# namascar/correlation

Hardware: AMD Instinct MI355X
Metric: correlation-point-iterations/sec (higher is better)
Workload: dtype f32

## Files before the change

### correlation_amd/build.py

```python
import os
import subprocess
import sys

HERE = os.path.dirname(os.path.abspath(__file__))
CSRC = os.path.join(HERE, "csrc")
LIB = os.path.join(HERE, "liblk_engine.so")
SOURCES = ["lk_engine.cpp", "lk_tracker.cpp", "lk_group.cpp", "lk_image_io.cpp", "lk_kernels.hip", "lk_guess_search.cpp",
           "lk_guess_search.hip", "lk_backward.hip", "lk_reseed.cpp", "lk_reseed.hip",
           "lk_strain.cpp", "lk_strain.hip", "lk_uncertainty.cpp", "lk_uncertainty.hip",
           "lk_outlier.cpp", "lk_outlier.hip", "lk_track.cpp", "lk_track.hip",
           "lk_residual.cpp", "lk_residual.hip", "lk_pattern.cpp", "lk_pattern.hip",
           "lk_field.cpp", "lk_field.hip", "lk_znssd.cpp", "lk_znssd.hip"]
HEADERS = ["lk_device.hpp", "lk_roi.hpp", "lk_solver_common.hpp", "lk_compose.hpp", "lk_launch.hpp", "lk_neighbours.hpp", "lk_rect_walk.hpp", "lk_sector_eval.hpp", "lk_cell_grid.hpp", "lk_pass.hpp", "lk_strain.hpp", "lk_uncertainty.hpp", "lk_outlier.hpp", "lk_track.hpp", "lk_residual.hpp", "lk_pattern.hpp", "lk_field.hpp", "lk_znssd.hpp", os.path.join("..", "..", "include", "lk_engine.h"),
           os.path.join("..", "..", "include", "lk_tracker.h"), os.path.join("..", "..", "include", "lk_group.h")]


def hipcc_path():
    for cand in (os.environ.get("HIPCC"), "/opt/rocm/bin/hipcc", "hipcc"):
        if cand and (os.path.isabs(cand) and os.path.exists(cand) or not os.path.isabs(cand)):
            return cand
    raise RuntimeError("hipcc not found")


def needs_build():
    if not os.path.exists(LIB):
        return True
    t = os.path.getmtime(LIB)
    deps = [os.path.join(CSRC, f) for f in SOURCES + HEADERS] + [os.path.abspath(__file__)]
    return any(os.path.getmtime(d) > t for d in deps if os.path.exists(d))


def build(force=False, verbose=False):
    if not force and not needs_build():
        return LIB
    from concurrent.futures import ThreadPoolExecutor
    objdir = os.path.join(os.path.dirname(HERE), "build", "obj")
    os.makedirs(objdir, exist_ok=True)
    flags = [
        "-O3", "--offload-arch=gfx950", "-fPIC", "-std=c++17",
        "-ffp-contract=off", "-fhip-fp32-correctly-rounded-divide-sqrt",
        "-fno-slp-vectorize",
        "-Wall", "-Wextra",
    ] + os.environ.get("LK_EXTRA_HIPCC_FLAGS", "").split()
    if verbose:
        flags.insert(0, "-Rpass-analysis=kernel-resource-usage")
    tag = os.path.join(objdir, "flags.txt")
    same_flags = os.path.exists(tag) and open(tag).read() == " ".join(flags)
    hdr_time = max(os.path.getmtime(os.path.join(CSRC, h)) for h in HEADERS + ["lk_internal.hpp"] if os.path.exists(os.path.join(CSRC, h)))

    def compile_one(src):
        obj = os.path.join(objdir, src + ".o")
        src_path = os.path.join(CSRC, src)
        if (not force and same_flags and os.path.exists(obj)
                and os.path.getmtime(obj) > max(os.path.getmtime(src_path), hdr_time)):
            return obj, None
        r = subprocess.run([hipcc_path()] + flags + ["-c", src, "-o", obj], cwd=CSRC, capture_output=True, text=True)
        return obj, r

    with ThreadPoolExecutor(max_workers=len(SOURCES)) as pool:
        results = list(pool.map(compile_one, SOURCES))
    for obj, r in results:
        if r is not None and r.returncode != 0:
            sys.stderr.write(r.stdout + r.stderr)
            raise RuntimeError("hipcc failed building " + os.path.basename(obj))
        if r is not None and verbose:
            sys.stderr.write(r.stderr)
    with open(tag, "w") as f:
        f.write(" ".join(flags))
    link = [hipcc_path(), "--offload-arch=gfx950", "-fPIC", "-shared", "-o", LIB] + [o for o, _ in results] + [
        "-lrocprofiler-sdk-roctx",
        "-lrccl",
        "-lz",
    ]
    r = subprocess.run(link, cwd=CSRC, capture_output=True, text=True)
    if r.returncode != 0:
        sys.stderr.write(r.stdout + r.stderr)
        raise RuntimeError("hipcc failed linking liblk_engine.so")
    return LIB


if __name__ == "__main__":
    print(build(force="--force" in sys.argv, verbose="-v" in sys.argv))
```

### correlation_amd/csrc/lk_kernels.hip

```cpp
#include "lk_device.hpp"
#include "lk_launch.hpp"

#include <float.h>
#include <stdlib.h>

#include <atomic>

#include "lk_rect_walk.hpp"
#include "lk_solver_common.hpp"

namespace {

struct LevelCtx {
  gptr<uint8_t> und, def;
  gptr<f32x2> xy;
  int rx, ry, rw;
  int n;
  int urows, ucols, drows, dcols;
  float cx, cy, scaling;
};

__device__ __forceinline__ float row16_sum(float v) {
  v = dpp_add<0xB1>(v);
  v = dpp_add<0x4E>(v);
// ... 1999 lines not shown
#pragma unroll
    for (int k = 0; k < 6; ++k)
      pr[k] = ps[k] = q[30 + k];
    const bool fr = damped_step<6, false>(S, lambda, scaling, pr, false, xr);
    const bool fs = damped_step_scattered(q[mine], q[mine + 1], lambda, scaling, ps, xs);
    bool same = __builtin_amdgcn_readfirstlane((int)fs) == (int)fs;
#pragma unroll
    for (int k = 0; k < 6; ++k)
      same = same && __builtin_amdgcn_readfirstlane((int)__float_as_uint(xs[k])) == (int)__float_as_uint(xs[k]) &&
             __builtin_amdgcn_readfirstlane((int)__float_as_uint(ps[k])) == (int)__float_as_uint(ps[k]);
    const bool all_same = __ballot(same) == ~0ull;
    if (l == 0) {
      float *o = out + (size_t)i * 32;
#pragma unroll
      for (int k = 0; k < 6; ++k) {
        o[k] = xr[k];
        o[6 + k] = pr[k];
        o[16 + k] = xs[k];
        o[22 + k] = ps[k];
      }
      o[12] = fr ? 1.f : 0.f;
      o[28] = fs ? 1.f : 0.f;
      o[13] = o[14] = o[15] = o[30] = o[31] = 0.f;
      o[29] = all_same ? 1.f : 0.f;
    }
  }
}

template <int N> __device__ __forceinline__ void row16_all_reduce(float (&v)[N]) {
#pragma unroll
  for (int i = 0; i < N; ++i)
    v[i] = dpp_add<0xB1>(v[i]);
#pragma unroll
  for (int i = 0; i < N; ++i)
    v[i] = dpp_add<0x4E>(v[i]);
#pragma unroll
  for (int i = 0; i < N; ++i)
    v[i] = dpp_add<0x141>(v[i]);
#pragma unroll
  for (int i = 0; i < N; ++i)
    v[i] = dpp_add<0x140>(v[i]);
}

template <int N> __device__ __forceinline__ void partner_rows_all_reduce(float (&v)[N], bool wide) {
#pragma unroll
  for (int i = 0; i < N; ++i)
    v[i] += __shfl_xor(v[i], 16, 64);
  if (wide) {
#pragma unroll
    for (int i = 0; i < N; ++i)
      v[i] += __shfl_xor(v[i], 32, 64);
  }
}

__global__ void __launch_bounds__(kWave) lk_reduce_compare_kernel(const float *in, float *out, int n, int wide) {
  const int l = (int)threadIdx.x;
  for (int i = (int)blockIdx.x; i < n; i += (int)gridDim.x) {
    const float *q = in + ((size_t)i * kWave + (size_t)l) * 28;
    float v[28], t[28];
#pragma unroll
    for (int k = 0; k < 28; ++k)
      v[k] = t[k] = q[k];
    row16_all_reduce(v);
    partner_rows_all_reduce(v, wide != 0);
    float s0, s1;
    row16_reduce_scatter28(t, s0, s1);
    s0 = add_partner_row(s0);
    s1 = add_partner_row(s1);
    if (wide) {
      s0 = add_partner_half(s0);
      s1 = add_partner_half(s1);
    }
    float g[28];
    gather_scattered(g, s0, s1, std::make_integer_sequence<int, 28>{});
    float *o = out + ((size_t)i * 2 * kWave + (size_t)l) * 28;
#pragma unroll
    for (int k = 0; k < 28; ++k) {
      o[k] = v[k];
      o[(size_t)kWave * 28 + k] = g[k];
    }
  }
}

__global__ void __launch_bounds__(256) lk_pyramid_kernel(const uint8_t *__restrict__ src,
                                                         int srows, int scols,
                                                         uint8_t *__restrict__ dst) {
  const int tcols = scols / 2, trows = srows / 2;
  const int tj = (int)(blockIdx.y * blockDim.y + threadIdx.y);
  const int ti0 = (int)(blockIdx.x * blockDim.x + threadIdx.x) * 4;
  if (tj >= trows || ti0 >= tcols)
    return;
  const float km[5] = {0.05f, 0.25f, 0.4f, 0.25f, 0.05f};
  float acc[4] = {0.f, 0.f, 0.f, 0.f};
  const bool row_inside = tj >= 1 && tj < trows - 1;
  const bool fast = 2 * ti0 - 4 >= 0 && 2 * ti0 + 12 <= scols;
  if (row_inside) {
#pragma unroll
    for (int dj = -2; dj <= 2; ++dj) {
      gptr<uint8_t> row = (gptr<uint8_t>)src + (size_t)(2 * tj + dj) * (size_t)scols;
      float px[11];
      if (fast) {
        const uint32_t w0 = load_u32_unaligned(row + 2 * ti0 - 4), w1 = load_u32_unaligned(row + 2 * ti0);
        const uint32_t w2 = load_u32_unaligned(row + 2 * ti0 + 4), w3 = load_u32_unaligned(row + 2 * ti0 + 8);
        px[0] = ub2(w0);
        px[1] = ub3(w0);
        px[2] = ub0(w1);
        px[3] = ub1(w1);
        px[4] = ub2(w1);
        px[5] = ub3(w1);
        px[6] = ub0(w2);
        px[7] = ub1(w2);
        px[8] = ub2(w2);
        px[9] = ub3(w2);
        px[10] = ub0(w3);
      } else {
#pragma unroll
        for (int c = 0; c < 11; ++c) {
          int sc = 2 * ti0 - 2 + c;
          sc = min(max(sc, 0), scols - 1);
          px[c] = (float)row[sc];
        }
      }
#pragma unroll
      for (int t = 0; t < 4; ++t)
#pragma unroll
        for (int di = 0; di < 5; ++di)
          acc[t] += px[2 * t + di] * (km[di] * km[dj + 2]);
    }
  }
  uint8_t o[4];
#pragma unroll
  for (int t = 0; t < 4; ++t) {
    const int ti = ti0 + t;
    const bool inside = row_inside && ti >= 1 && ti < tcols - 1;
    o[t] = inside ? (uint8_t)acc[t] : (uint8_t)0;
  }
  uint8_t *out = dst + (size_t)tj * (size_t)tcols + (size_t)ti0;
  if (ti0 + 4 <= tcols && (tcols & 3) == 0) {
    *reinterpret_cast<uint32_t *>(out) = (uint32_t)o[0] | ((uint32_t)o[1] << 8) | ((uint32_t)o[2] << 16) | ((uint32_t)o[3] << 24);
  } else {
#pragma unroll
    for (int t = 0; t < 4; ++t)
      if (ti0 + t < tcols)
        out[t] = o[t];
  }
}

struct LkLevelTable {
  LkLevelView v[LK_MAX_LEVELS];
};
__global__ void lk_set_views_kernel(LkLevelTable t, LkLevelView *out) {
  if (threadIdx.x < LK_MAX_LEVELS)
    out[threadIdx.x] = t.v[threadIdx.x];
}

constexpr int kPyrT0 = 64, kPyrR0 = 73, kPyrPitch0 = 80, kPyrR1 = 35, kPyrPitch1 = 36;

__device__ __forceinline__ uint8_t pyr_tap(const uint8_t *win, int pitch) {
  const float km[5] = {0.05f, 0.25f, 0.4f, 0.25f, 0.05f};
  float acc = 0.f;
#pragma unroll
  for (int dj = 0; dj < 5; ++dj)
#pragma unroll
    for (int di = 0; di < 5; ++di)
      acc += (float)win[dj * pitch + di] * (km[di] * km[dj]);
  return (uint8_t)acc;
}

struct LkPyrJobs {
  const uint8_t *src[2];
  int step[2];
  uint8_t *l0[2], *l1[2], *l2[2];
};

__global__ void __launch_bounds__(256) lk_pyramid2_kernel(LkPyrJobs jobs, int rows, int cols) {
  const uint8_t *src = jobs.src[blockIdx.z];
  const int step = jobs.step[blockIdx.z];
  uint8_t *l0 = jobs.l0[blockIdx.z], *l1 = jobs.l1[blockIdx.z], *l2 = jobs.l2[blockIdx.z];
  __shared__ __attribute__((aligned(16))) uint8_t s0[kPyrR0 * kPyrPitch0];
  __shared__ __attribute__((aligned(16))) uint8_t s1[kPyrR1 * kPyrPitch1];
  const int rows1 = rows / 2, cols1 = cols / 2, rows2 = rows1 / 2, cols2 = cols1 / 2;
  const int x2 = (int)blockIdx.x * 16, y2 = (int)blockIdx.y * 16;
  const int X0 = 4 * x2 - 8, Y0 = 4 * y2 - 6;
  const int tid = (int)threadIdx.x;
  const bool copy0 = src != l0;
  const bool dwords = ((reinterpret_cast<uintptr_t>(src) | (uintptr_t)step) & 3u) == 0 && (cols & 3) == 0;
  for (int i = tid; i < kPyrR0 * (kPyrPitch0 / 4); i += 256) {
    const int r = i / (kPyrPitch0 / 4), cw = i % (kPyrPitch0 / 4);
    const int gy = Y0 + r, gx = X0 + 4 * cw;
    uint32_t v = 0;
    if (gy >= 0 && gy < rows) {
      const uint8_t *row = src + (size_t)gy * (size_t)step;
      if (dwords && gx >= 0 && gx + 4 <= cols) {
        v = *reinterpret_cast<const uint32_t *>(row + gx);
      } else {
#pragma unroll
        for (int b = 0; b < 4; ++b)
          if (gx + b >= 0 && gx + b < cols)
            v |= (uint32_t)row[gx + b] << (8 * b);
      }
      if (copy0 && r >= 6 && r < 6 + kPyrT0 && cw >= 2 && cw < 2 + kPyrT0 / 4) {
        uint8_t *out = l0 + (size_t)gy * (size_t)cols + (size_t)gx;
        if ((cols & 3) == 0 && gx + 4 <= cols) {
          *reinterpret_cast<uint32_t *>(out) = v;
        } else {
#pragma unroll
          for (int b = 0; b < 4; ++b)
            if (gx + b < cols)
              out[b] = (uint8_t)(v >> (8 * b));
        }
      }
    }
    reinterpret_cast<uint32_t *>(s0)[i] = v;
  }
  __syncthreads();
  for (int t = tid; t < kPyrR1 * (kPyrPitch1 / 4); t += 256) {
    const int j = t / (kPyrPitch1 / 4), i0 = 4 * (t % (kPyrPitch1 / 4));
    const float km[5] = {0.05f, 0.25f, 0.4f, 0.25f, 0.05f};
    float acc[4] = {0.f, 0.f, 0.f, 0.f};
#pragma unroll
    for (int dj = 0; dj < 5; ++dj) {
      const uint2 *w = reinterpret_cast<const uint2 *>(s0 + (2 * j + dj) * kPyrPitch0 + 2 * i0);
      const uint2 a = w[0], b = w[1];
      const float px[11] = {ub2(a.x), ub3(a.x), ub0(a.y), ub1(a.y), ub2(a.y), ub3(a.y),
                            ub0(b.x), ub1(b.x), ub2(b.x), ub3(b.x), ub0(b.y)};
#pragma unroll
      for (int q = 0; q < 4; ++q)
#pragma unroll
        for (int di = 0; di < 5; ++di)
          acc[q] += px[2 * q + di] * (km[di] * km[dj]);
    }
    const int gj = 2 * y2 - 2 + j;
    uint32_t packed = 0;
#pragma unroll
    for (int q = 0; q < 4; ++q) {
      const int gi = 2 * x2 - 2 + i0 + q;
      const bool inside = gj >= 1 && gj < rows1 - 1 && gi >= 1 && gi < cols1 - 1;
      const uint32_t v = inside ? (uint32_t)(uint8_t)acc[q] : 0u;
      packed |= v << (8 * q);
      if (j >= 2 && j < 34 && i0 + q >= 2 && i0 + q < 34 && gj < rows1 && gi < cols1)
        l1[(size_t)gj * (size_t)cols1 + (size_t)gi] = (uint8_t)v;
    }
    *reinterpret_cast<uint32_t *>(s1 + j * kPyrPitch1 + i0) = packed;
  }
  __syncthreads();
  {
    const int j = tid / 16, i = tid % 16;
    const int gj = y2 + j, gi = x2 + i;
    if (gj < rows2 && gi < cols2) {
      const bool inside = gj >= 1 && gj < rows2 - 1 && gi >= 1 && gi < cols2 - 1;
      l2[(size_t)gj * (size_t)cols2 + (size_t)gi] =
          inside ? pyr_tap(s1 + (2 * j) * kPyrPitch1 + 2 * i, kPyrPitch1) : (uint8_t)0;
    }
  }
}

struct LkGuessArgs {
  const float2 *center;
  const float *last_p;
  float *prev_p;
  float *guess;
  float global_guess[6];
  float gcx, gcy;
  int n_sectors, model, frame, constant_velocity;
};

__global__ void lk_guess_kernel(LkGuessArgs a) {
  int s = (int)(blockIdx.x * blockDim.x + threadIdx.x);
  if (s >= a.n_sectors)
    return;
  const int P = n_params(a.model);
  float g[6] = {0, 0, 0, 0, 0, 0};
  if (a.frame == 0) {
    for (int i = 0; i < P; ++i)
      g[i] = a.global_guess[i];
    float2 c = a.center[s];
    float dx = c.x - a.gcx, dy = c.y - a.gcy;
    if (a.model == LK_FM_UVUXUYVXVY) {
      g[0] += dx * a.global_guess[2] + dy * a.global_guess[3];
      g[1] += dx * a.global_guess[4] + dy * a.global_guess[5];
    } else {
      float Vx = a.global_guess[2];
      g[0] += -dy * Vx;
      g[1] += dx * Vx;
    }
    for (int i = 0; i < 6; ++i)
      a.prev_p[(size_t)s * 6 + i] = i < P ? g[i] : 0.f;
  } else {
    for (int i = 0; i < P; ++i) {
      float r = a.last_p[(size_t)s * 6 + i], q = a.prev_p[(size_t)s * 6 + i];
      g[i] = a.constant_velocity ? r + (r - q) : r;
      a.prev_p[(size_t)s * 6 + i] = r;
    }
  }
  for (int i = 0; i < 6; ++i)
    a.guess[(size_t)s * 6 + i] = i < P ? g[i] : 0.f;
}

__global__ void lk_warp_points_kernel(const float2 *xy, int n, float cx, float cy, int model,
                                      const float *pp, float2 *out) {
  int k = (int)(blockIdx.x * blockDim.x + threadIdx.x);
  if (k >= n)
    return;
  float p[6];
  for (int i = 0; i < 6; ++i)
    p[i] = pp[i];
  float2 q = xy[k];
  float xd, yd, dx, dy;
  switch (model) {
  case LK_FM_U: Warp<LK_FM_U>::apply(q.x, q.y, cx, cy, p, xd, yd, dx, dy); break;
  case LK_FM_UV: Warp<LK_FM_UV>::apply(q.x, q.y, cx, cy, p, xd, yd, dx, dy); break;
  case LK_FM_UVQ: Warp<LK_FM_UVQ>::apply(q.x, q.y, cx, cy, p, xd, yd, dx, dy); break;
  default: Warp<LK_FM_UVUXUYVXVY>::apply(q.x, q.y, cx, cy, p, xd, yd, dx, dy); break;
  }
  out[k] = make_float2(xd, yd);
}


__device__ __forceinline__ int round_like_host(float v) {
  const float t = v + 0.5f;
  return fabsf(t) < 2147483648.f ? (int)t : (int)0x80000000;
}

template <int MODEL> __global__ void lk_rewarp_kernel(LkRewarpArgs a) {
  const uint32_t i = blockIdx.x * blockDim.x + threadIdx.x;
  if (i >= a.total)
    return;
  int lo = 0, hi = a.n_sectors;
  while (hi - lo > 1) {
    const int mid = (lo + hi) >> 1;
    if (a.dst_off[mid] <= i)
      lo = mid;
    else
      hi = mid;
  }
  const int s = lo;
  const uint32_t k = i - a.dst_off[s];
// ... 942 lines not shown
  }
}

hipError_t lk_launch_solve_seq(const LkSolveArgs &a, int model, int interp, int group, int flavour, hipStream_t st) {
  if (a.n_sectors <= 0 || a.seq_frames <= 0)
    return hipSuccess;
  if ((long long)a.n_sectors * a.seq_frames >= (1ll << 31) - (1ll << 20))
    return hipErrorInvalidValue;
  switch (model) {
#ifndef LK_TUNE_ONLY_AFFINE_BICUBIC
  case LK_FM_U: return launch_solve_seq_m<LK_FM_U>(a, interp, group, flavour, st);
  case LK_FM_UV: return launch_solve_seq_m<LK_FM_UV>(a, interp, group, flavour, st);
  case LK_FM_UVQ: return launch_solve_seq_m<LK_FM_UVQ>(a, interp, group, flavour, st);
#endif
  default: return launch_solve_seq_m<LK_FM_UVUXUYVXVY>(a, interp, group, flavour, st);
  }
}

template <int MODEL, int GROUP>
static hipError_t launch_eval_mg(const LkEvalArgs &a, int interp, hipStream_t st) {
  switch (interp) {
  case LK_IM_NEAREST: hipLaunchKernelGGL((lk_eval_kernel<MODEL, LK_IM_NEAREST, GROUP>), dim3(1), dim3(256), 0, st, a); break;
  case LK_IM_BILINEAR: hipLaunchKernelGGL((lk_eval_kernel<MODEL, LK_IM_BILINEAR, GROUP>), dim3(1), dim3(256), 0, st, a); break;
  case LK_IM_BICUBIC_SEPARABLE: hipLaunchKernelGGL((lk_eval_kernel<MODEL, LK_IM_BICUBIC_SEPARABLE, GROUP>), dim3(1), dim3(256), 0, st, a); break;
  default: hipLaunchKernelGGL((lk_eval_kernel<MODEL, LK_IM_BICUBIC, GROUP>), dim3(1), dim3(256), 0, st, a); break;
  }
  return hipGetLastError();
}

template <int MODEL>
static hipError_t launch_eval_m(const LkEvalArgs &a, int interp, int group, hipStream_t st) {
  switch (group) {
  case 16: return launch_eval_mg<MODEL, 16>(a, interp, st);
  case 32: return launch_eval_mg<MODEL, 32>(a, interp, st);
  case 64: return launch_eval_mg<MODEL, 64>(a, interp, st);
  default: return launch_eval_mg<MODEL, 256>(a, interp, st);
  }
}

hipError_t lk_launch_eval(const LkEvalArgs &a, int model, int interp, int group, hipStream_t st) {
  switch (model) {
  case LK_FM_U: return launch_eval_m<LK_FM_U>(a, interp, group, st);
  case LK_FM_UV: return launch_eval_m<LK_FM_UV>(a, interp, group, st);
  case LK_FM_UVQ: return launch_eval_m<LK_FM_UVQ>(a, interp, group, st);
  default: return launch_eval_m<LK_FM_UVUXUYVXVY>(a, interp, group, st);
  }
}

hipError_t lk_launch_step_compare(int n, const float *d_in, float *d_out, hipStream_t st) {
  hipLaunchKernelGGL(lk_step_compare_kernel, dim3(n < 256 ? n : 256), dim3(kWave), 0, st, d_in, d_out, n);
  return hipGetLastError();
}

hipError_t lk_launch_reduce_compare(int n, int wide, const float *d_in, float *d_out, hipStream_t st) {
  hipLaunchKernelGGL(lk_reduce_compare_kernel, dim3(n < 256 ? n : 256), dim3(kWave), 0, st, d_in, d_out, n, wide);
  return hipGetLastError();
}

hipError_t lk_launch_solve_only(int n, const float *d_in, float *d_out, hipStream_t st) {
  switch (n) {
  case 1: hipLaunchKernelGGL((lk_solve_only_kernel<1>), dim3(1), dim3(64), 0, st, d_in, d_out); break;
  case 2: hipLaunchKernelGGL((lk_solve_only_kernel<2>), dim3(1), dim3(64), 0, st, d_in, d_out); break;
  case 3: hipLaunchKernelGGL((lk_solve_only_kernel<3>), dim3(1), dim3(64), 0, st, d_in, d_out); break;
  case 6: hipLaunchKernelGGL((lk_solve_only_kernel<6>), dim3(1), dim3(64), 0, st, d_in, d_out); break;
  default: return hipErrorInvalidValue;
  }
  return hipGetLastError();
}

hipError_t lk_launch_sample(int interp, const uint8_t *def, int rows, int cols, const float2 *pts, int n,
                            float4 *out, hipStream_t st) {
  if (n <= 0)
    return hipSuccess;
  dim3 grid((unsigned)((n + 255) / 256)), block(256);
  switch (interp) {
  case LK_IM_NEAREST: hipLaunchKernelGGL((lk_sample_kernel<LK_IM_NEAREST>), grid, block, 0, st, def, rows, cols, pts, n, out); break;
  case LK_IM_BILINEAR: hipLaunchKernelGGL((lk_sample_kernel<LK_IM_BILINEAR>), grid, block, 0, st, def, rows, cols, pts, n, out); break;
  case LK_IM_BICUBIC_SEPARABLE: hipLaunchKernelGGL((lk_sample_kernel<LK_IM_BICUBIC_SEPARABLE>), grid, block, 0, st, def, rows, cols, pts, n, out); break;
  default: hipLaunchKernelGGL((lk_sample_kernel<LK_IM_BICUBIC>), grid, block, 0, st, def, rows, cols, pts, n, out); break;
  }
  return hipGetLastError();
}

hipError_t lk_launch_pyramid(const uint8_t *src, int srows, int scols, uint8_t *dst, hipStream_t st) {
  int tcols = scols / 2, trows = srows / 2;
  if (tcols <= 0 || trows <= 0)
    return hipSuccess;
  dim3 block(64, 4);
  dim3 grid((unsigned)((tcols + 4 * 64 - 1) / (4 * 64)), (unsigned)((trows + 3) / 4));
  hipLaunchKernelGGL(lk_pyramid_kernel, grid, block, 0, st, src, srows, scols, dst);
  return hipGetLastError();
}

hipError_t lk_launch_set_views(const LkLevelView *h_views, LkLevelView *d_views, hipStream_t st) {
  LkLevelTable t;
  for (int l = 0; l < LK_MAX_LEVELS; ++l)
    t.v[l] = h_views[l];
  hipLaunchKernelGGL(lk_set_views_kernel, dim3(1), dim3(64), 0, st, t, d_views);
  return hipGetLastError();
}

hipError_t lk_launch_pyramid2(int n_images, const uint8_t *const *src, const int *step, int rows, int cols,
                              uint8_t *const *l0, uint8_t *const *l1, uint8_t *const *l2, hipStream_t st) {
  if (rows / 4 <= 0 || cols / 4 <= 0 || n_images < 1 || n_images > 2)
    return hipErrorInvalidValue;
  LkPyrJobs jobs{};
  for (int i = 0; i < n_images; ++i) {
    jobs.src[i] = src[i];
    jobs.step[i] = step[i];
    jobs.l0[i] = l0[i];
    jobs.l1[i] = l1[i];
    jobs.l2[i] = l2[i];
  }
  dim3 grid((unsigned)((cols + kPyrT0 - 1) / kPyrT0), (unsigned)((rows + kPyrT0 - 1) / kPyrT0), (unsigned)n_images);
  hipLaunchKernelGGL(lk_pyramid2_kernel, grid, dim3(256), 0, st, jobs, rows, cols);
  return hipGetLastError();
}

hipError_t lk_launch_guess(const float2 *center, const float *last_p, float *prev_p, float *guess,
                           const float *global_guess, float gcx, float gcy, int n_sectors, int model,
                           int frame, int constant_velocity, hipStream_t st) {
  LkGuessArgs a;
  a.center = center;
  a.last_p = last_p;
  a.prev_p = prev_p;
  a.guess = guess;
  for (int i = 0; i < 6; ++i)
    a.global_guess[i] = global_guess[i];
  a.gcx = gcx;
  a.gcy = gcy;
  a.n_sectors = n_sectors;
  a.model = model;
  a.frame = frame;
  a.constant_velocity = constant_velocity;
  if (n_sectors <= 0)
    return hipSuccess;
  hipLaunchKernelGGL(lk_guess_kernel, dim3((unsigned)((n_sectors + 255) / 256)), dim3(256), 0, st, a);
  return hipGetLastError();
}

hipError_t lk_launch_warp_points(const float2 *xy, int n, float cx, float cy, int model, const float *d_p,
                                 float2 *out, hipStream_t st) {
  if (n <= 0)
    return hipSuccess;
  hipLaunchKernelGGL(lk_warp_points_kernel, dim3((unsigned)((n + 255) / 256)), dim3(256), 0, st, xy, n, cx,
                     cy, model, d_p, out);
  return hipGetLastError();
}

hipError_t lk_launch_rewarp(const LkRewarpArgs &a, int model, hipStream_t st) {
  if (a.total == 0)
    return hipSuccess;
  const dim3 grid((a.total + 255) / 256), block(256);
  switch (model) {
  case LK_FM_U: hipLaunchKernelGGL(lk_rewarp_kernel<LK_FM_U>, grid, block, 0, st, a); break;
  case LK_FM_UV: hipLaunchKernelGGL(lk_rewarp_kernel<LK_FM_UV>, grid, block, 0, st, a); break;
  case LK_FM_UVQ: hipLaunchKernelGGL(lk_rewarp_kernel<LK_FM_UVQ>, grid, block, 0, st, a); break;
  default: hipLaunchKernelGGL(lk_rewarp_kernel<LK_FM_UVUXUYVXVY>, grid, block, 0, st, a); break;
  }
  return hipGetLastError();
}

int lk_decimate_tiles(uint32_t n_max) { return (int)((n_max + kScanTile - 1) / kScanTile); }

hipError_t lk_launch_decimate(const float2 *xy_prev, const uint32_t *off_prev, const uint32_t *n_prev, uint32_t n_max,
                              int level_delta, int n_sectors, uint32_t *pos, uint32_t *tiles, float2 *xy_out,
                              uint32_t *off_out, uint32_t *n_out, hipStream_t st) {
  const int mag = 1 << level_delta, n_tiles = lk_decimate_tiles(n_max);
  if (n_tiles == 0)
    return hipSuccess;
  hipLaunchKernelGGL(lk_decimate_flag_kernel, dim3((unsigned)n_tiles), dim3(kScanThreads), 0, st, xy_prev, n_prev, mag,
                     pos, tiles);
  hipLaunchKernelGGL(lk_scan_tiles_kernel, dim3(1), dim3(1024), 0, st, tiles, n_tiles, n_out);
  hipLaunchKernelGGL(lk_decimate_scatter_kernel, dim3((n_max + kScanThreads - 1) / kScanThreads), dim3(kScanThreads), 0,
                     st, xy_prev, n_prev, 1.f / (float)mag, pos, tiles, xy_out);
  hipLaunchKernelGGL(lk_decimate_offsets_kernel, dim3((unsigned)(n_sectors + 256) / 256), dim3(256), 0, st, off_prev,
                     n_prev, pos, tiles, n_tiles, n_sectors, off_out);
  return hipGetLastError();
}

static_assert(kLkRoiTile == kScanTile, "one ROI tile = one pass of the block scan");

hipError_t lk_launch_roi_count(const LkRoiSector *sectors, const LkRoiFlat *flats, const uint32_t *tile_begin, int n_sectors,
                               uint32_t n_tiles, uint32_t *tiles, uint32_t *n_out, hipStream_t st, int rows) {
  if (n_tiles == 0)
    return hipSuccess;
  if (rows)
    hipLaunchKernelGGL((lk_roi_tile_kernel<false, true>), dim3(n_tiles), dim3(kScanThreads), 0, st, sectors, flats, tile_begin,
                       n_sectors, tiles, (const uint32_t *)nullptr, (float2 *)nullptr);
  else
  hipLaunchKernelGGL(lk_roi_tile_kernel<false>, dim3(n_tiles), dim3(kScanThreads), 0, st, sectors, flats, tile_begin, n_sectors,
                     tiles, (const uint32_t *)nullptr, (float2 *)nullptr);
  hipLaunchKernelGGL(lk_scan_tiles_kernel, dim3(1), dim3(1024), 0, st, tiles, (int)n_tiles, n_out);
  return hipGetLastError();
}

hipError_t lk_launch_roi_fill(const LkRoiSector *sectors, const LkRoiFlat *flats, const uint32_t *tile_begin, int n_sectors,
                              uint32_t n_tiles, const uint32_t *tiles, float2 *xy, uint32_t *off, hipStream_t st, int rows) {
// ... 42 lines not shown
```

### correlation_amd/csrc/lk_launch.hpp

```cpp
#pragma once
#include <hip/hip_runtime.h>
#include <stddef.h>
#include <stdint.h>

#include "lk_device.hpp"

hipError_t lk_launch_solve(const LkSolveArgs &a, int model, int interp, int group, hipStream_t st);
hipError_t lk_launch_solve_seq(const LkSolveArgs &a, int model, int interp, int group, int flavour, hipStream_t st);
hipError_t lk_launch_eval(const LkEvalArgs &a, int model, int interp, int group, hipStream_t st);
hipError_t lk_launch_solve_only(int n, const float *d_in, float *d_out, hipStream_t st);
hipError_t lk_launch_step_compare(int n, const float *d_in, float *d_out, hipStream_t st);
hipError_t lk_launch_reduce_compare(int n, int wide, const float *d_in, float *d_out, hipStream_t st);
hipError_t lk_launch_sample(int interp, const uint8_t *def, int rows, int cols, const float2 *pts, int n,
                            float4 *out, hipStream_t st);

hipError_t lk_launch_backward(const LkBackwardArgs &a, int model, int interp, int group, hipStream_t st);
hipError_t lk_launch_backward_eval(const LkBackwardEvalArgs &a, int model, int interp, int group, hipStream_t st);

hipError_t lk_launch_guess_search(const LkGuessSearchArgs &a, hipStream_t st);
int lk_guess_search_window_budget(int radius, int has_v);

hipError_t lk_launch_pyramid(const uint8_t *src, int srows, int scols, uint8_t *dst, hipStream_t st);
hipError_t lk_launch_set_views(const LkLevelView *h_views, LkLevelView *d_views, hipStream_t st);
hipError_t lk_launch_pyramid2(int n_images, const uint8_t *const *src, const int *step, int rows, int cols,
                              uint8_t *const *l0, uint8_t *const *l1, uint8_t *const *l2, hipStream_t st);

hipError_t lk_launch_warp_points(const float2 *xy, int n, float cx, float cy, int model, const float *d_p,
                                 float2 *out, hipStream_t st);
hipError_t lk_launch_rewarp(const LkRewarpArgs &a, int model, hipStream_t st);
int lk_decimate_tiles(uint32_t n_max);
hipError_t lk_launch_decimate(const float2 *xy_prev, const uint32_t *off_prev, const uint32_t *n_prev, uint32_t n_max,
                              int level_delta, int n_sectors, uint32_t *pos, uint32_t *tiles, float2 *xy_out,
                              uint32_t *off_out, uint32_t *n_out, hipStream_t st);
hipError_t lk_launch_roi_count(const LkRoiSector *sectors, const LkRoiFlat *flats, const uint32_t *tile_begin, int n_sectors,
                               uint32_t n_tiles, uint32_t *tiles, uint32_t *n_out, hipStream_t st, int rows = 0);
hipError_t lk_launch_roi_fill(const LkRoiSector *sectors, const LkRoiFlat *flats, const uint32_t *tile_begin, int n_sectors,
                              uint32_t n_tiles, const uint32_t *tiles, float2 *xy, uint32_t *off, hipStream_t st, int rows = 0);
hipError_t lk_launch_mean_center(const float2 *xy, const uint32_t *off, int n_sectors, float2 *center, hipStream_t st);
size_t lk_mean_center_int_scratch_bytes(uint32_t n_samples, int n_sectors);
hipError_t lk_launch_mean_center_int(const float2 *xy, const uint32_t *off, uint32_t n_samples, int n_sectors, void *scratch,
                                     float2 *center, hipStream_t st);

hipError_t lk_launch_guess(const float2 *center, const float *last_p, float *prev_p, float *guess,
                           const float *global_guess, float gcx, float gcy, int n_sectors, int model,
                           int frame, int constant_velocity, hipStream_t st);
hipError_t lk_launch_append_sector(const LkAppendArgs &a, hipStream_t st);
hipError_t lk_launch_stale_iterations(lk_result *r, int n, const int *carry_in, int *carry_out, hipStream_t st);
hipError_t lk_launch_stale_iterations_blocks(lk_result *all, int n_sectors, int n_ranks, int cap, const int *carry_in,
                                             int *carry_out, hipStream_t st);
hipError_t lk_launch_stale_iterations_window(lk_result *all, int n_sectors, int n_ranks, int cap, int frames, const int *carry_in,
                                             int *carry_out, hipStream_t st);

hipError_t lk_launch_reseed_bbox(const float2 *center, int n_sectors, float *out4, hipStream_t st);
hipError_t lk_launch_reseed_classify(const lk_result *rec, int n_sectors, int n_params, float chi_max, uint8_t *good,
                                     int32_t *tried, lk_reseed_info *info, uint32_t *n_failed, hipStream_t st);
hipError_t lk_launch_reseed_grid(const float2 *center, int n_sectors, double x0, double y0, double cell, int nx, int ny,
                                 uint32_t *cell_of, uint32_t *start, uint32_t *cursor, uint32_t *unordered, uint32_t *members,
                                 hipStream_t st);
hipError_t lk_launch_reseed_plan(const LkReseedPlanArgs &a, hipStream_t st);
hipError_t lk_launch_reseed_compact(const LkReseedCompactArgs &a, hipStream_t st);
hipError_t lk_launch_reseed_merge(const LkReseedMergeArgs &a, hipStream_t st);

hipError_t lk_launch_pack_prep(const lk_result *rec, const float2 *center, int n_sectors, int n_frames, int model, float chi_max,
                               int canonical_zero, uint8_t *good, float4 *pack, hipStream_t st);
hipError_t lk_launch_strain(const LkStrainArgs &a, int group, int packed, hipStream_t st);

hipError_t lk_launch_uncertainty(const LkUncertaintyArgs &a, int model, int interp, int group, hipStream_t st);

hipError_t lk_launch_outlier_exclude(const lk_outlier *flags, const float2 *center, const uint8_t *good, int n_sectors,
                                     float4 *pack, hipStream_t st);
hipError_t lk_launch_outlier(const LkOutlierArgs &a, int group, hipStream_t st);
hipError_t lk_launch_outlier_mark(const lk_outlier *flags, int n_sectors, lk_result *rec, hipStream_t st);

hipError_t lk_launch_track(const LkTrackArgs &a, int group, hipStream_t st);

hipError_t lk_launch_photometry(const LkPhotometryArgs &a, int model, int interp, int group, hipStream_t st);
hipError_t lk_launch_map_prep(const lk_result *rec, const float2 *center, int n_sectors, int model, int level, float chi_max,
                              LkMapSector *pack, hipStream_t st);
hipError_t lk_launch_residual_map(const LkResidualMapArgs &a, int model, int interp, int *n_tiles, hipStream_t st);

hipError_t lk_launch_znssd(const LkZnssdArgs &a, int model, int interp, int group, hipStream_t st);

hipError_t lk_launch_pattern(const LkPatternArgs &a, int group, hipStream_t st);
hipError_t lk_launch_sat_build(const LkSatArgs &a, hipStream_t st);
hipError_t lk_launch_subset_query(const LkSubsetArgs &a, hipStream_t st);

hipError_t lk_launch_field_map(const LkFieldArgs &a, int weight, int frame, int *n_tiles, hipStream_t st);
```

Baseline: 488.6 million.

## Move pyramid kernels to own file and restructure fused pyramid2 staging

Measured after the change: 492.7 million, median of 6. Within noise of the previous version (+0.8%).

```diff
diff --git a/correlation_amd/build.py b/correlation_amd/build.py
--- a/correlation_amd/build.py
+++ b/correlation_amd/build.py
@@ -5,7 +5,7 @@
 HERE = os.path.dirname(os.path.abspath(__file__))
 CSRC = os.path.join(HERE, "csrc")
 LIB = os.path.join(HERE, "liblk_engine.so")
-SOURCES = ["lk_engine.cpp", "lk_tracker.cpp", "lk_group.cpp", "lk_image_io.cpp", "lk_kernels.hip", "lk_guess_search.cpp",
+SOURCES = ["lk_engine.cpp", "lk_tracker.cpp", "lk_group.cpp", "lk_image_io.cpp", "lk_kernels.hip", "lk_pyramid.hip", "lk_guess_search.cpp",
            "lk_guess_search.hip", "lk_backward.hip", "lk_reseed.cpp", "lk_reseed.hip",
            "lk_strain.cpp", "lk_strain.hip", "lk_uncertainty.cpp", "lk_uncertainty.hip",
            "lk_outlier.cpp", "lk_outlier.hip", "lk_track.cpp", "lk_track.hip",
diff --git a/correlation_amd/csrc/lk_kernels.hip b/correlation_amd/csrc/lk_kernels.hip
--- a/correlation_amd/csrc/lk_kernels.hip
+++ b/correlation_amd/csrc/lk_kernels.hip
@@ -2105,177 +2105,12 @@
   }
 }
 
-__global__ void __launch_bounds__(256) lk_pyramid_kernel(const uint8_t *__restrict__ src,
-                                                         int srows, int scols,
-                                                         uint8_t *__restrict__ dst) {
-  const int tcols = scols / 2, trows = srows / 2;
-  const int tj = (int)(blockIdx.y * blockDim.y + threadIdx.y);
-  const int ti0 = (int)(blockIdx.x * blockDim.x + threadIdx.x) * 4;
-  if (tj >= trows || ti0 >= tcols)
-    return;
-  const float km[5] = {0.05f, 0.25f, 0.4f, 0.25f, 0.05f};
-  float acc[4] = {0.f, 0.f, 0.f, 0.f};
-  const bool row_inside = tj >= 1 && tj < trows - 1;
-  const bool fast = 2 * ti0 - 4 >= 0 && 2 * ti0 + 12 <= scols;
-  if (row_inside) {
-#pragma unroll
-    for (int dj = -2; dj <= 2; ++dj) {
-      gptr<uint8_t> row = (gptr<uint8_t>)src + (size_t)(2 * tj + dj) * (size_t)scols;
-      float px[11];
-      if (fast) {
-        const uint32_t w0 = load_u32_unaligned(row + 2 * ti0 - 4), w1 = load_u32_unaligned(row + 2 * ti0);
-        const uint32_t w2 = load_u32_unaligned(row + 2 * ti0 + 4), w3 = load_u32_unaligned(row + 2 * ti0 + 8);
-        px[0] = ub2(w0);
-        px[1] = ub3(w0);
-        px[2] = ub0(w1);
-        px[3] = ub1(w1);
-        px[4] = ub2(w1);
-        px[5] = ub3(w1);
-        px[6] = ub0(w2);
-        px[7] = ub1(w2);
-        px[8] = ub2(w2);
-        px[9] = ub3(w2);
-        px[10] = ub0(w3);
-      } else {
-#pragma unroll
-        for (int c = 0; c < 11; ++c) {
-          int sc = 2 * ti0 - 2 + c;
-          sc = min(max(sc, 0), scols - 1);
-          px[c] = (float)row[sc];
-        }
-      }
-#pragma unroll
-      for (int t = 0; t < 4; ++t)
-#pragma unroll
-        for (int di = 0; di < 5; ++di)
-          acc[t] += px[2 * t + di] * (km[di] * km[dj + 2]);
-    }
-  }
-  uint8_t o[4];
-#pragma unroll
-  for (int t = 0; t < 4; ++t) {
-    const int ti = ti0 + t;
-    const bool inside = row_inside && ti >= 1 && ti < tcols - 1;
-    o[t] = inside ? (uint8_t)acc[t] : (uint8_t)0;
-  }
-  uint8_t *out = dst + (size_t)tj * (size_t)tcols + (size_t)ti0;
-  if (ti0 + 4 <= tcols && (tcols & 3) == 0) {
-    *reinterpret_cast<uint32_t *>(out) = (uint32_t)o[0] | ((uint32_t)o[1] << 8) | ((uint32_t)o[2] << 16) | ((uint32_t)o[3] << 24);
-  } else {
-#pragma unroll
-    for (int t = 0; t < 4; ++t)
-      if (ti0 + t < tcols)
-        out[t] = o[t];
-  }
-}
-
 struct LkLevelTable {
   LkLevelView v[LK_MAX_LEVELS];
 };
 __global__ void lk_set_views_kernel(LkLevelTable t, LkLevelView *out) {
   if (threadIdx.x < LK_MAX_LEVELS)
     out[threadIdx.x] = t.v[threadIdx.x];
-}
-
-constexpr int kPyrT0 = 64, kPyrR0 = 73, kPyrPitch0 = 80, kPyrR1 = 35, kPyrPitch1 = 36;
-
-__device__ __forceinline__ uint8_t pyr_tap(const uint8_t *win, int pitch) {
-  const float km[5] = {0.05f, 0.25f, 0.4f, 0.25f, 0.05f};
-  float acc = 0.f;
-#pragma unroll
-  for (int dj = 0; dj < 5; ++dj)
-#pragma unroll
-    for (int di = 0; di < 5; ++di)
-      acc += (float)win[dj * pitch + di] * (km[di] * km[dj]);
-  return (uint8_t)acc;
-}
-
-struct LkPyrJobs {
-  const uint8_t *src[2];
-  int step[2];
-  uint8_t *l0[2], *l1[2], *l2[2];
-};
-
-__global__ void __launch_bounds__(256) lk_pyramid2_kernel(LkPyrJobs jobs, int rows, int cols) {
-  const uint8_t *src = jobs.src[blockIdx.z];
-  const int step = jobs.step[blockIdx.z];
-  uint8_t *l0 = jobs.l0[blockIdx.z], *l1 = jobs.l1[blockIdx.z], *l2 = jobs.l2[blockIdx.z];
-  __shared__ __attribute__((aligned(16))) uint8_t s0[kPyrR0 * kPyrPitch0];
-  __shared__ __attribute__((aligned(16))) uint8_t s1[kPyrR1 * kPyrPitch1];
-  const int rows1 = rows / 2, cols1 = cols / 2, rows2 = rows1 / 2, cols2 = cols1 / 2;
-  const int x2 = (int)blockIdx.x * 16, y2 = (int)blockIdx.y * 16;
-  const int X0 = 4 * x2 - 8, Y0 = 4 * y2 - 6;
-  const int tid = (int)threadIdx.x;
-  const bool copy0 = src != l0;
-  const bool dwords = ((reinterpret_cast<uintptr_t>(src) | (uintptr_t)step) & 3u) == 0 && (cols & 3) == 0;
-  for (int i = tid; i < kPyrR0 * (kPyrPitch0 / 4); i += 256) {
-    const int r = i / (kPyrPitch0 / 4), cw = i % (kPyrPitch0 / 4);
-    const int gy = Y0 + r, gx = X0 + 4 * cw;
-    uint32_t v = 0;
-    if (gy >= 0 && gy < rows) {
-      const uint8_t *row = src + (size_t)gy * (size_t)step;
-      if (dwords && gx >= 0 && gx + 4 <= cols) {
-        v = *reinterpret_cast<const uint32_t *>(row + gx);
-      } else {
-#pragma unroll
-        for (int b = 0; b < 4; ++b)
-          if (gx + b >= 0 && gx + b < cols)
-            v |= (uint32_t)row[gx + b] << (8 * b);
-      }
-      if (copy0 && r >= 6 && r < 6 + kPyrT0 && cw >= 2 && cw < 2 + kPyrT0 / 4) {
-        uint8_t *out = l0 + (size_t)gy * (size_t)cols + (size_t)gx;
-        if ((cols & 3) == 0 && gx + 4 <= cols) {
-          *reinterpret_cast<uint32_t *>(out) = v;
-        } else {
-#pragma unroll
-          for (int b = 0; b < 4; ++b)
-            if (gx + b < cols)
-              out[b] = (uint8_t)(v >> (8 * b));
-        }
-      }
-    }
-    reinterpret_cast<uint32_t *>(s0)[i] = v;
-  }
-  __syncthreads();
-  for (int t = tid; t < kPyrR1 * (kPyrPitch1 / 4); t += 256) {
-    const int j = t / (kPyrPitch1 / 4), i0 = 4 * (t % (kPyrPitch1 / 4));
-    const float km[5] = {0.05f, 0.25f, 0.4f, 0.25f, 0.05f};
-    float acc[4] = {0.f, 0.f, 0.f, 0.f};
-#pragma unroll
-    for (int dj = 0; dj < 5; ++dj) {
-      const uint2 *w = reinterpret_cast<const uint2 *>(s0 + (2 * j + dj) * kPyrPitch0 + 2 * i0);
-      const uint2 a = w[0], b = w[1];
-      const float px[11] = {ub2(a.x), ub3(a.x), ub0(a.y), ub1(a.y), ub2(a.y), ub3(a.y),
-                            ub0(b.x), ub1(b.x), ub2(b.x), ub3(b.x), ub0(b.y)};
-#pragma unroll
-      for (int q = 0; q < 4; ++q)
-#pragma unroll
-        for (int di = 0; di < 5; ++di)
-          acc[q] += px[2 * q + di] * (km[di] * km[dj]);
-    }
-    const int gj = 2 * y2 - 2 + j;
-    uint32_t packed = 0;
-#pragma unroll
-    for (int q = 0; q < 4; ++q) {
-      const int gi = 2 * x2 - 2 + i0 + q;
-      const bool inside = gj >= 1 && gj < rows1 - 1 && gi >= 1 && gi < cols1 - 1;
-      const uint32_t v = inside ? (uint32_t)(uint8_t)acc[q] : 0u;
-      packed |= v << (8 * q);
-      if (j >= 2 && j < 34 && i0 + q >= 2 && i0 + q < 34 && gj < rows1 && gi < cols1)
-        l1[(size_t)gj * (size_t)cols1 + (size_t)gi] = (uint8_t)v;
-    }
-    *reinterpret_cast<uint32_t *>(s1 + j * kPyrPitch1 + i0) = packed;
-  }
-  __syncthreads();
-  {
-    const int j = tid / 16, i = tid % 16;
-    const int gj = y2 + j, gi = x2 + i;
-    if (gj < rows2 && gi < cols2) {
-      const bool inside = gj >= 1 && gj < rows2 - 1 && gi >= 1 && gi < cols2 - 1;
-      l2[(size_t)gj * (size_t)cols2 + (size_t)gi] =
-          inside ? pyr_tap(s1 + (2 * j) * kPyrPitch1 + 2 * i, kPyrPitch1) : (uint8_t)0;
-    }
-  }
 }
 
 struct LkGuessArgs {
@@ -3384,38 +3219,11 @@
   return hipGetLastError();
 }
 
-hipError_t lk_launch_pyramid(const uint8_t *src, int srows, int scols, uint8_t *dst, hipStream_t st) {
-  int tcols = scols / 2, trows = srows / 2;
-  if (tcols <= 0 || trows <= 0)
-    return hipSuccess;
-  dim3 block(64, 4);
-  dim3 grid((unsigned)((tcols + 4 * 64 - 1) / (4 * 64)), (unsigned)((trows + 3) / 4));
-  hipLaunchKernelGGL(lk_pyramid_kernel, grid, block, 0, st, src, srows, scols, dst);
-  return hipGetLastError();
-}
-
 hipError_t lk_launch_set_views(const LkLevelView *h_views, LkLevelView *d_views, hipStream_t st) {
   LkLevelTable t;
   for (int l = 0; l < LK_MAX_LEVELS; ++l)
     t.v[l] = h_views[l];
   hipLaunchKernelGGL(lk_set_views_kernel, dim3(1), dim3(64), 0, st, t, d_views);
-  return hipGetLastError();
-}
-
-hipError_t lk_launch_pyramid2(int n_images, const uint8_t *const *src, const int *step, int rows, int cols,
-                              uint8_t *const *l0, uint8_t *const *l1, uint8_t *const *l2, hipStream_t st) {
-  if (rows / 4 <= 0 || cols / 4 <= 0 || n_images < 1 || n_images > 2)
-    return hipErrorInvalidValue;
-  LkPyrJobs jobs{};
-  for (int i = 0; i < n_images; ++i) {
-    jobs.src[i] = src[i];
-    jobs.step[i] = step[i];
-    jobs.l0[i] = l0[i];
-    jobs.l1[i] = l1[i];
-    jobs.l2[i] = l2[i];
-  }
-  dim3 grid((unsigned)((cols + kPyrT0 - 1) / kPyrT0), (unsigned)((rows + kPyrT0 - 1) / kPyrT0), (unsigned)n_images);
-  hipLaunchKernelGGL(lk_pyramid2_kernel, grid, dim3(256), 0, st, jobs, rows, cols);
   return hipGetLastError();
 }
 
diff --git a/correlation_amd/csrc/lk_launch.hpp b/correlation_amd/csrc/lk_launch.hpp
--- a/correlation_amd/csrc/lk_launch.hpp
+++ b/correlation_amd/csrc/lk_launch.hpp
@@ -21,9 +21,10 @@
 int lk_guess_search_window_budget(int radius, int has_v);
 
 hipError_t lk_launch_pyramid(const uint8_t *src, int srows, int scols, uint8_t *dst, hipStream_t st);
-hipError_t lk_launch_set_views(const LkLevelView *h_views, LkLevelView *d_views, hipStream_t st);
 hipError_t lk_launch_pyramid2(int n_images, const uint8_t *const *src, const int *step, int rows, int cols,
                               uint8_t *const *l0, uint8_t *const *l1, uint8_t *const *l2, hipStream_t st);
+
+hipError_t lk_launch_set_views(const LkLevelView *h_views, LkLevelView *d_views, hipStream_t st);
 
 hipError_t lk_launch_warp_points(const float2 *xy, int n, float cx, float cy, int model, const float *d_p,
                                  float2 *out, hipStream_t st);
diff --git a/correlation_amd/csrc/lk_pyramid.hip b/correlation_amd/csrc/lk_pyramid.hip
--- /dev/null
+++ b/correlation_amd/csrc/lk_pyramid.hip
@@ -0,0 +1,235 @@
+#include "lk_device.hpp"
+#include "lk_launch.hpp"
+
+#include "lk_solver_common.hpp"
+
+namespace {
+
+__global__ void __launch_bounds__(256) lk_pyramid_kernel(const uint8_t *__restrict__ src,
+                                                         int srows, int scols,
+                                                         uint8_t *__restrict__ dst) {
+  const int tcols = scols / 2, trows = srows / 2;
+  const int tj = (int)(blockIdx.y * blockDim.y + threadIdx.y);
+  const int ti0 = (int)(blockIdx.x * blockDim.x + threadIdx.x) * 4;
+  if (tj >= trows || ti0 >= tcols)
+    return;
+  const float km[5] = {0.05f, 0.25f, 0.4f, 0.25f, 0.05f};
+  float acc[4] = {0.f, 0.f, 0.f, 0.f};
+  const bool row_inside = tj >= 1 && tj < trows - 1;
+  const bool fast = 2 * ti0 - 4 >= 0 && 2 * ti0 + 12 <= scols;
+  if (row_inside) {
+#pragma unroll
+    for (int dj = -2; dj <= 2; ++dj) {
+      gptr<uint8_t> row = (gptr<uint8_t>)src + (size_t)(2 * tj + dj) * (size_t)scols;
+      float px[11];
+      if (fast) {
+        const uint32_t w0 = load_u32_unaligned(row + 2 * ti0 - 4), w1 = load_u32_unaligned(row + 2 * ti0);
+        const uint32_t w2 = load_u32_unaligned(row + 2 * ti0 + 4), w3 = load_u32_unaligned(row + 2 * ti0 + 8);
+        px[0] = ub2(w0);
+        px[1] = ub3(w0);
+        px[2] = ub0(w1);
+        px[3] = ub1(w1);
+        px[4] = ub2(w1);
+        px[5] = ub3(w1);
+        px[6] = ub0(w2);
+        px[7] = ub1(w2);
+        px[8] = ub2(w2);
+        px[9] = ub3(w2);
+        px[10] = ub0(w3);
+      } else {
+#pragma unroll
+        for (int c = 0; c < 11; ++c) {
+          int sc = 2 * ti0 - 2 + c;
+          sc = min(max(sc, 0), scols - 1);
+          px[c] = (float)row[sc];
+        }
+      }
+#pragma unroll
+      for (int t = 0; t < 4; ++t)
+#pragma unroll
+        for (int di = 0; di < 5; ++di)
+          acc[t] += px[2 * t + di] * (km[di] * km[dj + 2]);
+    }
+  }
+  uint8_t o[4];
+#pragma unroll
+  for (int t = 0; t < 4; ++t) {
+    const int ti = ti0 + t;
+    const bool inside = row_inside && ti >= 1 && ti < tcols - 1;
+    o[t] = inside ? (uint8_t)acc[t] : (uint8_t)0;
+  }
+  uint8_t *out = dst + (size_t)tj * (size_t)tcols + (size_t)ti0;
+  if (ti0 + 4 <= tcols && (tcols & 3) == 0) {
+    *reinterpret_cast<uint32_t *>(out) = (uint32_t)o[0] | ((uint32_t)o[1] << 8) | ((uint32_t)o[2] << 16) | ((uint32_t)o[3] << 24);
+  } else {
+#pragma unroll
+    for (int t = 0; t < 4; ++t)
+      if (ti0 + t < tcols)
+        out[t] = o[t];
+  }
+}
+
+constexpr int kPyrT0 = 64;
+constexpr int kPyrR0 = 73, kPyrPitch0 = 80;
+constexpr int kPyrW0 = kPyrPitch0 / 4;
+constexpr int kPyrStage = (kPyrR0 * kPyrW0 + 255) / 256;
+constexpr int kPyrR1 = 35, kPyrPitch1 = 40;
+constexpr int kPyrTasks1 = kPyrR1 * 9;
+
+template <int PITCH> __device__ __forceinline__ void pyr_tap4(const uint8_t *win, float (&acc)[4]) {
+  const float km[5] = {0.05f, 0.25f, 0.4f, 0.25f, 0.05f};
+#pragma unroll
+  for (int q = 0; q < 4; ++q)
+    acc[q] = 0.f;
+#pragma unroll
+  for (int dj = 0; dj < 5; ++dj) {
+    const uint2 *w = reinterpret_cast<const uint2 *>(win + dj * PITCH);
+    const uint2 a = w[0], b = w[1];
+    const float px[11] = {ub2(a.x), ub3(a.x), ub0(a.y), ub1(a.y), ub2(a.y), ub3(a.y),
+                          ub0(b.x), ub1(b.x), ub2(b.x), ub3(b.x), ub0(b.y)};
+#pragma unroll
+    for (int q = 0; q < 4; ++q)
+#pragma unroll
+      for (int di = 0; di < 5; ++di)
+        acc[q] += px[2 * q + di] * (km[di] * km[dj]);
+  }
+}
+
+__device__ __forceinline__ uint32_t pyr_pack4(const float (&acc)[4], int gj, int gi0, int rows_t, int cols_t) {
+  const bool row_inside = gj >= 1 && gj < rows_t - 1;
+  uint32_t packed = 0;
+#pragma unroll
+  for (int q = 0; q < 4; ++q) {
+    const int gi = gi0 + q;
+    const bool inside = row_inside && gi >= 1 && gi < cols_t - 1;
+    packed |= (inside ? (uint32_t)(uint8_t)acc[q] : 0u) << (8 * q);
+  }
+  return packed;
+}
+
+__device__ __forceinline__ void pyr_store4(uint8_t *out, uint32_t v, int gi0, int cols_t) {
+  if ((cols_t & 3) == 0) {
+    *reinterpret_cast<uint32_t *>(out) = v;
+  } else {
+#pragma unroll
+    for (int b = 0; b < 4; ++b)
+      if (gi0 + b < cols_t)
+        out[b] = (uint8_t)(v >> (8 * b));
+  }
+}
+
+struct LkPyrJobs {
+  const uint8_t *src[2];
+  int step[2];
+  uint8_t *l0[2], *l1[2], *l2[2];
+};
+
+__global__ void __launch_bounds__(256) lk_pyramid2_kernel(LkPyrJobs jobs, int rows, int cols) {
+  const uint8_t *src = jobs.src[blockIdx.z];
+  const int step = jobs.step[blockIdx.z];
+  uint8_t *l0 = jobs.l0[blockIdx.z], *l1 = jobs.l1[blockIdx.z], *l2 = jobs.l2[blockIdx.z];
+  __shared__ __attribute__((aligned(16))) uint8_t s0[kPyrR0 * kPyrPitch0];
+  __shared__ __attribute__((aligned(16))) uint8_t s1[kPyrR1 * kPyrPitch1];
+  const int rows1 = rows / 2, cols1 = cols / 2, rows2 = rows1 / 2, cols2 = cols1 / 2;
+  const int x2 = (int)blockIdx.x * 16, y2 = (int)blockIdx.y * 16;
+  const int X0 = 4 * x2 - 8, Y0 = 4 * y2 - 6;
+  const int tid = (int)threadIdx.x, wave = tid >> 6, lane = tid & 63;
+  const bool copy0 = src != l0;
+  const bool dwords = ((reinterpret_cast<uintptr_t>(src) | (uintptr_t)step) & 3u) == 0 && (cols & 3) == 0;
+  int r[kPyrStage], cw[kPyrStage];
+  r[0] = tid / kPyrW0;
+  cw[0] = tid - r[0] * kPyrW0;
+#pragma unroll
+  for (int k = 1; k < kPyrStage; ++k) {
+    const int c = cw[k - 1] + 256 % kPyrW0;
+    r[k] = r[k - 1] + 256 / kPyrW0 + (c >= kPyrW0);
+    cw[k] = c >= kPyrW0 ? c - kPyrW0 : c;
+  }
+  uint32_t v[kPyrStage];
+  if (dwords) {
+#pragma unroll
+    for (int k = 0; k < kPyrStage; ++k) {
+      const int gy = min(max(Y0 + r[k], 0), rows - 1), gx = min(max(X0 + 4 * cw[k], 0), cols - 4);
+      v[k] = *reinterpret_cast<const uint32_t *>(src + (size_t)gy * (size_t)step + (size_t)gx);
+    }
+  } else {
+#pragma unroll
+    for (int k = 0; k < kPyrStage; ++k) {
+      const uint8_t *row = src + (size_t)min(max(Y0 + r[k], 0), rows - 1) * (size_t)step;
+      uint32_t b[4];
+#pragma unroll
+      for (int q = 0; q < 4; ++q)
+        b[q] = row[min(max(X0 + 4 * cw[k] + q, 0), cols - 1)];
+      v[k] = b[0] | (b[1] << 8) | (b[2] << 16) | (b[3] << 24);
+    }
+  }
+#pragma unroll
+  for (int k = 0; k < kPyrStage; ++k) {
+    if (r[k] < kPyrR0) {
+      reinterpret_cast<uint32_t *>(s0)[tid + 256 * k] = v[k];
+      const int gy = Y0 + r[k], gx = X0 + 4 * cw[k];
+      if (copy0 && r[k] >= 6 && r[k] < 6 + kPyrT0 && cw[k] >= 2 && cw[k] < 2 + kPyrT0 / 4 && gy < rows && gx < cols)
+        pyr_store4(l0 + (size_t)gy * (size_t)cols + (size_t)gx, v[k], gx, cols);
+    }
+  }
+  __syncthreads();
+#pragma unroll 1
+  for (int pass = 0; pass < 2; ++pass) {
+    const int t = pass == 0 ? tid : wave == 0 ? 256 + lane : kPyrTasks1;
+    if (t >= kPyrTasks1)
+      continue;
+    const int j = t / 9, i0 = 4 * (t - 9 * j);
+    float acc[4];
+    pyr_tap4<kPyrPitch0>(s0 + (2 * j) * kPyrPitch0 + 2 * i0, acc);
+    const uint32_t packed = pyr_pack4(acc, 2 * y2 - 2 + j, 2 * x2 - 2 + i0, rows1, cols1);
+    uint16_t *o = reinterpret_cast<uint16_t *>(s1 + j * kPyrPitch1 + i0 + 2);
+    o[0] = (uint16_t)packed;
+    o[1] = (uint16_t)(packed >> 16);
+  }
+  __syncthreads();
+  {
+    const int j = tid >> 3, g = tid & 7;
+    const int gj = 2 * y2 + j, gi0 = 2 * x2 + 4 * g;
+    if (gj < rows1 && gi0 < cols1)
+      pyr_store4(l1 + (size_t)gj * (size_t)cols1 + (size_t)gi0, *reinterpret_cast<const uint32_t *>(s1 + (j + 2) * kPyrPitch1 + 4 + 4 * g),
+                 gi0, cols1);
+  }
+  if (wave == 2) {
+    const int j = lane >> 2, i0 = 4 * (lane & 3);
+    const int gj = y2 + j, gi0 = x2 + i0;
+    if (gj < rows2 && gi0 < cols2) {
+      float acc[4];
+      pyr_tap4<kPyrPitch1>(s1 + (2 * j) * kPyrPitch1 + 2 * i0, acc);
+      pyr_store4(l2 + (size_t)gj * (size_t)cols2 + (size_t)gi0, pyr_pack4(acc, gj, gi0, rows2, cols2), gi0, cols2);
+    }
+  }
+}
+
+}
+
+hipError_t lk_launch_pyramid(const uint8_t *src, int srows, int scols, uint8_t *dst, hipStream_t st) {
+  int tcols = scols / 2, trows = srows / 2;
+  if (tcols <= 0 || trows <= 0)
+    return hipSuccess;
+  dim3 block(64, 4);
+  dim3 grid((unsigned)((tcols + 4 * 64 - 1) / (4 * 64)), (unsigned)((trows + 3) / 4));
+  hipLaunchKernelGGL(lk_pyramid_kernel, grid, block, 0, st, src, srows, scols, dst);
+  return hipGetLastError();
+}
+
+hipError_t lk_launch_pyramid2(int n_images, const uint8_t *const *src, const int *step, int rows, int cols,
+                              uint8_t *const *l0, uint8_t *const *l1, uint8_t *const *l2, hipStream_t st) {
+  if (rows / 4 <= 0 || cols / 4 <= 0 || n_images < 1 || n_images > 2)
+    return hipErrorInvalidValue;
+  LkPyrJobs jobs{};
+  for (int i = 0; i < n_images; ++i) {
+    jobs.src[i] = src[i];
+    jobs.step[i] = step[i];
+    jobs.l0[i] = l0[i];
+    jobs.l1[i] = l1[i];
+    jobs.l2[i] = l2[i];
+  }
+  dim3 grid((unsigned)((cols + kPyrT0 - 1) / kPyrT0), (unsigned)((rows + kPyrT0 - 1) / kPyrT0), (unsigned)n_images);
+  hipLaunchKernelGGL(lk_pyramid2_kernel, grid, dim3(256), 0, st, jobs, rows, cols);
+  return hipGetLastError();
+}
```
